# nanoporetech/medaka

Measured on NVIDIA H100. Metric: pileup positions/sec (consensus inference), higher is better.
Workload: dtype f32

## Files before the change

### medaka_b200/csrc/gru_wg.cu

```cuda
#include "common.cuh"
#include "ptx.cuh"
#include "rec_common.cuh"

namespace mdk {

constexpr int RW_THREADS = 256;
constexpr int RW_ABLK = (H / 8) * 64 * 16;
constexpr int RW_XBLK = 2 * 64 * 16;

template <int NT, bool FUSE_X, int OUT>
struct RwCfg {
    static constexpr int N = NT * RT_N;
    static constexpr bool HL = NT == 1;
    static constexpr int ROWS = HL ? 2 * N : N;
    static constexpr int PLANES = HL ? 1 : 2;
    static constexpr int KG = ROWS * 16 + 16;
    static_assert(KG % 16 == 0, "stmatrix rows are 16-byte aligned");
    static constexpr int HPLANE = (H / 8) * KG;
    static constexpr int XPLANE = 2 * KG;
    static constexpr int HLO = HL ? N * 16 : HPLANE;
    static constexpr int XLO = HL ? N * 16 : XPLANE;
    static constexpr int RED = (RW_THREADS / 32) * NCLS * N;
    static constexpr int wlo_off = 0;
    static constexpr int wxlo_off = wlo_off + 6 * RW_ABLK;
    static constexpr int h_off = wxlo_off + (FUSE_X ? 6 * RW_XBLK : 0);
    static constexpr int x_off = h_off + 2 * PLANES * HPLANE;
    static constexpr int red_off = x_off + (FUSE_X ? 2 * PLANES * XPLANE : 0);
    static constexpr int total = red_off + (OUT == OUT_LOGITS ? 2 * RED * 4 : 0);
    static_assert(total <= 227 * 1024, "smem budget");
};

__device__ __forceinline__ uint32_t ld_u32(const __half *p) { return *reinterpret_cast<const uint32_t *>(p); }

template <int NT, bool FUSE_X, int OUT>
__global__ void __launch_bounds__(RW_THREADS, 1)
rec_tc_kernel(const float *__restrict__ gi, RecX xin, const __half *__restrict__ w_hh, const float *__restrict__ b_hn,
              void *__restrict__ h_out, int64_t B, int64_t T, const float *__restrict__ lin_w,
              float *__restrict__ plog) {
    using L = RwCfg<NT, FUSE_X, OUT>;
    constexpr int N = L::N, NA = N / 2;
    constexpr int NACC = L::ROWS / 2;
    constexpr int NX = FUSE_X ? NACC : NA;
    using MMA = Wgmma<N>;
    using MMA_H = Wgmma<L::ROWS>;
    constexpr bool LOGITS = OUT == OUT_LOGITS;
    extern __shared__ __align__(128) uint8_t smem[];
    const int tid = threadIdx.x, wg = tid >> 7, warp = (tid >> 5) & 3, lane = tid & 31;
    const int gq = lane >> 2, cq = lane & 3;
    const int dir = blockIdx.y;
    const int64_t ntiles = (B + RT_N - 1) / RT_N;
    const int64_t wtile0 = (int64_t)blockIdx.x * NT;
    const int j0 = wg * 64 + warp * 16 + gq;
    const uint32_t sbase = smem_u32(smem);

    for (int i = tid; i < (L::total - L::h_off) / 16; i += RW_THREADS)
        reinterpret_cast<int4 *>(smem + L::h_off)[i] = make_int4(0, 0, 0, 0);
    for (int i = tid; i < 3 * H * (H / 8); i += RW_THREADS) {
        const int kg = i & 15, r = (i >> 4) & (H - 1), gate = i >> 11;
        const uint4 v = *reinterpret_cast<const uint4 *>(w_hh + ((((size_t)dir * 2 + 1) * 3 + gate) * H + r) * H + kg * 8);
        *reinterpret_cast<uint4 *>(smem + L::wlo_off + (gate * 2 + (r >> 6)) * RW_ABLK + kg * 1024 + (r & 63) * 16) = v;
    }
    if (FUSE_X) {
        for (int i = tid; i < 3 * H * 2; i += RW_THREADS) {
            const int kg = i & 1, r = (i >> 1) & (H - 1), gate = i >> 8;
            const uint4 v = *reinterpret_cast<const uint4 *>(xin.w_x + ((((size_t)dir * 2 + 1) * 3 + gate) * H + r) * 16 + kg * 8);
            *reinterpret_cast<uint4 *>(smem + L::wxlo_off + (gate * 2 + (r >> 6)) * RW_XBLK + kg * 1024 + (r & 63) * 16) = v;
        }
    }
    float wlin[2][NCLS];
    if (LOGITS) {
#pragma unroll
        for (int hb = 0; hb < 2; ++hb)
#pragma unroll
            for (int c = 0; c < NCLS; ++c) wlin[hb][c] = lin_w[c * H2 + dir * H + j0 + 8 * hb];
    }
    uint32_t whi[3][H / 16][4];
#pragma unroll
    for (int gate = 0; gate < 3; ++gate)
#pragma unroll
        for (int ks = 0; ks < H / 16; ++ks) {
            const __half *w = w_hh + ((((size_t)dir * 2) * 3 + gate) * H + j0) * H + ks * 16 + 2 * cq;
            whi[gate][ks][0] = ld_u32(w);
            whi[gate][ks][1] = ld_u32(w + 8 * H);
            whi[gate][ks][2] = ld_u32(w + 8);
            whi[gate][ks][3] = ld_u32(w + 8 * H + 8);
        }
    uint32_t wxhi[3][4];
    float bx[3][2] = {};
    if (FUSE_X) {
#pragma unroll
        for (int gate = 0; gate < 3; ++gate) {
            const __half *w = xin.w_x + ((((size_t)dir * 2) * 3 + gate) * H + j0) * 16 + 2 * cq;
            wxhi[gate][0] = ld_u32(w);
            wxhi[gate][1] = ld_u32(w + 8 * 16);
            wxhi[gate][2] = ld_u32(w + 8);
            wxhi[gate][3] = ld_u32(w + 8 * 16 + 8);
            bx[gate][0] = xin.bias[dir * G3 + gate * H + j0];
            bx[gate][1] = xin.bias[dir * G3 + gate * H + j0 + 8];
        }
    }
    const float bhn[2] = {b_hn[dir * H + j0], b_hn[dir * H + j0 + 8]};
    const uint32_t hst_addr = sbase + L::h_off + (lane >> 4) * L::HLO + (wg * 8 + warp * 2 + ((lane >> 3) & 1)) * L::KG +
                              (lane & 7) * 16;

    float ar[NACC], az[NACC], an[NACC], axn[NX], hp[NA];
#pragma unroll
    for (int k = 0; k < NA; ++k) hp[k] = 0.f;
    const float *gi_thr = FUSE_X ? nullptr
                                 : gi + wtile0 * T * GI_TS_FLOATS + ((dir * 3 * 4 + (cq >> 1)) * H + j0) * 4 + 2 * (cq & 1);
    auto load_pre = [&](int64_t t) {
#pragma unroll
        for (int i = 0; i < N / 8; ++i)
#pragma unroll
            for (int hb = 0; hb < 2; ++hb) {
                float2 v[3] = {make_float2(0.f, 0.f), make_float2(0.f, 0.f), make_float2(0.f, 0.f)};
                if (FUSE_X) {
#pragma unroll
                    for (int gate = 0; gate < 3; ++gate) v[gate] = make_float2(bx[gate][hb], bx[gate][hb]);
                } else if (i < 2 || wtile0 + (i >> 1) < ntiles) {
                    const float *p = gi_thr + ((i >> 1) * T + t) * GI_TS_FLOATS + (2 * (i & 1) * H + 8 * hb) * 4;
#pragma unroll
                    for (int gate = 0; gate < 3; ++gate) v[gate] = __ldcs(reinterpret_cast<const float2 *>(p + gate * 16 * H));
                }
                const int k = 4 * i + 2 * hb;
                ar[k] = v[0].x; ar[k + 1] = v[0].y;
                az[k] = v[1].x; az[k + 1] = v[1].y;
                axn[k] = v[2].x; axn[k + 1] = v[2].y;
                an[k] = bhn[hb]; an[k + 1] = bhn[hb];
            }
        if constexpr (L::HL) {
#pragma unroll
            for (int k = NA; k < NACC; ++k) {
                ar[k] = 0.f; az[k] = 0.f; an[k] = 0.f;
                if constexpr (FUSE_X) axn[k] = 0.f;
            }
        }
    };
    const int xF = FUSE_X ? xin.F : 1;
    const float *xsrc[NT];
    int xoff[NT];
    float xreg[NT];
#pragma unroll
    for (int m = 0; m < NT; ++m) {
        const int q = tid + RW_THREADS * m, xn = q / xF, xf = q - xn * xF;
        const bool own = FUSE_X && q < N * xF;
        xoff[m] = own ? (xf >> 3) * L::KG + xn * 16 + (xf & 7) * 2 : -1;
        xsrc[m] = (own && wtile0 * RT_N + xn < B) ? xin.feats + ((wtile0 * RT_N + xn) * T) * xF + xf : nullptr;
        xreg[m] = 0.f;
    }
    auto stage_x = [&](int buf, int m, float v) {
        __half hi, lo;
        split_f16(v, hi, lo);
        *reinterpret_cast<__half *>(smem + L::x_off + buf * L::PLANES * L::XPLANE + xoff[m]) = hi;
        *reinterpret_cast<__half *>(smem + L::x_off + buf * L::PLANES * L::XPLANE + L::XLO + xoff[m]) = lo;
    };
    const int64_t t_first = dir ? T - 1 : 0;
    if (FUSE_X) {
#pragma unroll
        for (int m = 0; m < NT; ++m) {
            if (xoff[m] < 0) continue;
            stage_x(0, m, xsrc[m] ? xsrc[m][t_first * xF] : 0.f);
        }
    }
    load_pre(t_first);
    fence_proxy_async_smem();
    __syncthreads();

    constexpr int NW = N / 4;
    auto head_partials = [&](int rb) {
        float v[NW][NCLS];
#pragma unroll
        for (int wl = 0; wl < NW; ++wl) {
            const int k = 4 * (wl >> 1) + (wl & 1);
#pragma unroll
            for (int c = 0; c < NCLS; ++c) v[wl][c] = fmaf(wlin[1][c], hp[k + 2], wlin[0][c] * hp[k]);
        }
        int wbase = 0;
#pragma unroll
        for (int lvl = 0; lvl < 3; ++lvl) {
            const int mask = 16 >> lvl;
            const int half = (NW >> lvl) / 2;
            if (half > 0) {
                const bool up = lane & mask;
#pragma unroll
                for (int w = 0; w < NW / 2; ++w) {
                    if (w >= half) continue;
#pragma unroll
                    for (int c = 0; c < NCLS; ++c) {
                        const float send = up ? v[w][c] : v[w + half][c];
                        const float keep = up ? v[w + half][c] : v[w][c];
                        v[w][c] = keep + __shfl_xor_sync(0xffffffffu, send, mask);
                    }
                }
                if (up) wbase += half;
            } else {
#pragma unroll
                for (int c = 0; c < NCLS; ++c) v[0][c] += __shfl_xor_sync(0xffffffffu, v[0][c], mask);
            }
        }
        if (NW >= 8 || !(lane & 4)) {
            float *red = reinterpret_cast<float *>(smem + L::red_off) + rb * L::RED + (tid >> 5) * NCLS * N;
            const int n = 8 * (wbase >> 1) + 2 * cq + (wbase & 1);
#pragma unroll
            for (int c = 0; c < NCLS; ++c) red[c * N + n] = v[0][c];
        }
    };
    auto head_store = [&](int rb, int64_t t) {
        if (tid >= NCLS * N) return;
        const int c = tid / N, n = tid % N;
        const float *red = reinterpret_cast<const float *>(smem + L::red_off) + rb * L::RED + c * N + n;
        float s = red[0];
#pragma unroll
        for (int w = 1; w < RW_THREADS / 32; ++w) s += red[w * NCLS * N];
        const int64_t wt = wtile0 + n / RT_N;
        if (wt < ntiles) plog[((dir * ntiles + wt) * T + t) * PLOG_TS_FLOATS + c * RT_N + (n & 15)] = s;
    };
    auto store_h0 = [&](int b, int64_t t) {
#pragma unroll
        for (int r = 0; r < NT * 512 / RW_THREADS; ++r) {
            const int q = tid + RW_THREADS * r, row = q & 15, kg = (q >> 4) & 15, p = (q >> 8) & 1, m = q >> 9;
            const int64_t wt = wtile0 + m;
            if (wt >= ntiles) continue;
            const int64_t orow = (wt * T + t) * RT_N + row;
            const int4 v = *reinterpret_cast<const int4 *>(smem + L::h_off + b * L::PLANES * L::HPLANE + p * L::HLO + kg * L::KG +
                                                           (m * RT_N + row) * 16);
            *reinterpret_cast<int4 *>(reinterpret_cast<uint8_t *>(h_out) + (orow >> 7) * (int64_t)XT_TILE_BYTES +
                                      p * XT_PLANE_BYTES + (dir * (H / 8) + kg) * (XT_ROWS * 16) + (orow & (XT_ROWS - 1)) * 16) = v;
        }
    };

#pragma unroll 1
    for (int64_t step = 0; step < T; ++step) {
        const int64_t t = dir ? T - 1 - step : step;
        const int buf = (int)(step & 1);
        const uint32_t hb_addr = sbase + L::h_off + buf * L::PLANES * L::HPLANE;
        wg_fence();
        if constexpr (L::HL) {
#pragma unroll
            for (int ks = 0; ks < H / 16; ++ks) {
                const uint64_t bh = make_smem_desc(hb_addr + ks * 2 * L::KG, L::KG, 128);
#pragma unroll
                for (int gate = 0; gate < 3; ++gate) MMA_H::rs(gate == 0 ? ar : (gate == 1 ? az : an), whi[gate][ks], bh, 1u);
#pragma unroll
                for (int gate = 0; gate < 3; ++gate)
                    MMA::ss(gate == 0 ? ar : (gate == 1 ? az : an),
                            make_smem_desc(sbase + L::wlo_off + (gate * 2 + wg) * RW_ABLK + ks * 2 * 1024, 1024, 128), bh, 1u);
            }
        } else {
#pragma unroll
            for (int ks = 0; ks < H / 16; ++ks) {
                const uint64_t bh = make_smem_desc(hb_addr + ks * 2 * L::KG, L::KG, 128);
                const uint64_t bl = make_smem_desc(hb_addr + L::HPLANE + ks * 2 * L::KG, L::KG, 128);
#pragma unroll
                for (int gate = 0; gate < 3; ++gate) MMA::rs(gate == 0 ? ar : (gate == 1 ? az : an), whi[gate][ks], bh, 1u);
#pragma unroll
                for (int gate = 0; gate < 3; ++gate) MMA::rs(gate == 0 ? ar : (gate == 1 ? az : an), whi[gate][ks], bl, 1u);
#pragma unroll
                for (int gate = 0; gate < 3; ++gate)
                    MMA::ss(gate == 0 ? ar : (gate == 1 ? az : an),
                            make_smem_desc(sbase + L::wlo_off + (gate * 2 + wg) * RW_ABLK + ks * 2 * 1024, 1024, 128), bh, 1u);
            }
        }
        if constexpr (FUSE_X) {
            const uint32_t xa = sbase + L::x_off + buf * L::PLANES * L::XPLANE;
            const uint64_t bh = make_smem_desc(xa, L::KG, 128);
            if constexpr (L::HL) {
#pragma unroll
                for (int gate = 0; gate < 3; ++gate) MMA_H::rs(gate == 0 ? ar : (gate == 1 ? az : axn), wxhi[gate], bh, 1u);
#pragma unroll
                for (int gate = 0; gate < 3; ++gate)
                    MMA::ss(gate == 0 ? ar : (gate == 1 ? az : axn),
                            make_smem_desc(sbase + L::wxlo_off + (gate * 2 + wg) * RW_XBLK, 1024, 128), bh, 1u);
            } else {
                const uint64_t bl = make_smem_desc(xa + L::XPLANE, L::KG, 128);
#pragma unroll
                for (int gate = 0; gate < 3; ++gate) MMA::rs(gate == 0 ? ar : (gate == 1 ? az : axn), wxhi[gate], bh, 1u);
#pragma unroll
                for (int gate = 0; gate < 3; ++gate) MMA::rs(gate == 0 ? ar : (gate == 1 ? az : axn), wxhi[gate], bl, 1u);
#pragma unroll
                for (int gate = 0; gate < 3; ++gate)
                    MMA::ss(gate == 0 ? ar : (gate == 1 ? az : axn),
                            make_smem_desc(sbase + L::wxlo_off + (gate * 2 + wg) * RW_XBLK, 1024, 128), bh, 1u);
            }
        }
        wg_commit();
        if (FUSE_X && step + 1 < T) {
#pragma unroll
            for (int m = 0; m < NT; ++m)
                if (xsrc[m]) xreg[m] = xsrc[m][(dir ? t - 1 : t + 1) * xF];
        }
        if (OUT == OUT_TILES && step > 0) store_h0(buf, dir ? t + 1 : t - 1);
        if (!FUSE_X && tid == 0 && step + GI_PREFETCH_STEPS < T) {
            const int64_t tp = dir ? t - GI_PREFETCH_STEPS : t + GI_PREFETCH_STEPS;
#pragma unroll
            for (int m = 0; m < NT; ++m) {
                if (wtile0 + m >= ntiles) break;
                const float *blk = gi + ((wtile0 + m) * T + tp) * GI_TS_FLOATS + (int64_t)dir * (GI_TS_FLOATS / 2);
#pragma unroll
                for (int i = 0; i < 12; ++i) bulk_prefetch_l2(blk + i * 512, 2048);
            }
        }
        if (LOGITS && step > 0) {
            if (step > 1) head_store((int)((step - 1) & 1), dir ? t + 2 : t - 2);
            head_partials((int)(step & 1));
        }
        wg_wait_all();
        wg_hold(ar); wg_hold(az); wg_hold(an); wg_hold(axn);

#pragma unroll
        for (int k = 0; k < NA; ++k) {
            float pr = ar[k], pz = az[k], pn = an[k], px = axn[k];
            if constexpr (L::HL) {
                pr += ar[k + NA]; pz += az[k + NA]; pn += an[k + NA];
                if constexpr (FUSE_X) px += axn[k + NA];
            }
            const float a = 1.f + ex2_approx(fminf(pr, EXP_CLAMP)), b = 1.f + ex2_approx(fminf(pz, EXP_CLAMP));
            const float q = rcp_approx(a * b);
            const float r = b * q, z = a * q;
            const float en = ex2_approx(fminf(fmaf(r, pn, px), EXP_CLAMP));
            const float n = (en - 1.f) * rcp_approx(en + 1.f);
            hp[k] = fmaf(z, hp[k] - n, n);
        }
#pragma unroll
        for (int i = 0; i < N / 8; ++i) {
            uint32_t hi[2], lo[2];
#pragma unroll
            for (int hb = 0; hb < 2; ++hb) split_f16x2(hp[4 * i + 2 * hb], hp[4 * i + 2 * hb + 1], hi[hb], lo[hb]);
            stmatrix_x4_trans(hst_addr + (buf ^ 1) * L::PLANES * L::HPLANE + i * 128, hi[0], hi[1], lo[0], lo[1]);
        }
        if (FUSE_X && step + 1 < T) {
#pragma unroll
            for (int m = 0; m < NT; ++m) {
                if (xoff[m] < 0) continue;
                stage_x(buf ^ 1, m, xreg[m]);
            }
        }
        if (OUT == OUT_ROWS) {
#pragma unroll
            for (int k = 0; k < NA; ++k) {
                const int i = k >> 2, n = 8 * i + 2 * cq + (k & 1);
                const int64_t wt = wtile0 + (i >> 1);
                if (wt >= ntiles) continue;
                const int64_t orow = (wt * T + t) * RT_N + (n & 15);
                reinterpret_cast<float *>(h_out)[orow * H2 + dir * H + j0 + 8 * ((k >> 1) & 1)] = hp[k];
            }
        }
        if (FUSE_X || step + 1 < T) load_pre(dir ? t - 1 : t + 1);
        fence_proxy_async_smem();
        __syncthreads();
    }
    if (OUT == OUT_TILES) store_h0((int)(T & 1), dir ? 0 : T - 1);
    if (LOGITS) {
        if (T > 1) head_store((int)((T - 1) & 1), dir ? 1 : T - 2);
        head_partials((int)(T & 1));
        __syncthreads();
        head_store((int)(T & 1), dir ? 0 : T - 1);
    }
}

template <int NT, bool FX, int OUT>
static cudaError_t launch_rec(const float *gi, const RecX &xin, const __half *w_hh_tm, const float *b_hn, void *out,
                              const float *lin_w, int64_t B, int64_t T, cudaStream_t s) {
    auto kern = rec_tc_kernel<NT, FX, OUT>;
    constexpr int smem_bytes = RwCfg<NT, FX, OUT>::total;
    cudaError_t e = cudaFuncSetAttribute(kern, cudaFuncAttributeMaxDynamicSharedMemorySize, smem_bytes);
    if (e != cudaSuccess) return e;
    const int64_t tiles = (B + RT_N - 1) / RT_N;
    dim3 grid((unsigned)((tiles + NT - 1) / NT), NDIR);
    constexpr bool LOGITS = OUT == OUT_LOGITS;
    kern<<<grid, RW_THREADS, smem_bytes, s>>>(gi, xin, w_hh_tm, b_hn, LOGITS ? nullptr : out, B, T, lin_w,
                                              LOGITS ? static_cast<float *>(out) : nullptr);
    return cudaGetLastError();
}

template <int NT>
static cudaError_t launch_rec_nt(const float *gi, const RecX *xin, const __half *w_hh_tm, const float *b_hn, int out_kind,
                                 void *out, const float *lin_w, int64_t B, int64_t T, cudaStream_t s) {
    if (xin)
        return out_kind == OUT_TILES ? launch_rec<NT, true, OUT_TILES>(gi, *xin, w_hh_tm, b_hn, out, nullptr, B, T, s)
                                     : cudaErrorInvalidValue;
    const RecX none{nullptr, nullptr, nullptr, 0};
    switch (out_kind) {
    case OUT_TILES: return launch_rec<NT, false, OUT_TILES>(gi, none, w_hh_tm, b_hn, out, nullptr, B, T, s);
    case OUT_ROWS: return launch_rec<NT, false, OUT_ROWS>(gi, none, w_hh_tm, b_hn, out, nullptr, B, T, s);
    case OUT_LOGITS:
        return lin_w ? launch_rec<NT, false, OUT_LOGITS>(gi, none, w_hh_tm, b_hn, out, lin_w, B, T, s) : cudaErrorInvalidValue;
    }
    return cudaErrorInvalidValue;
}

cudaError_t launch_rec_tc(const float *gi, const RecX *xin, const __half *w_hh_tm, const float *b_hn, int tiles_per_cta,
                          int out_kind, void *out, const float *lin_w, int64_t B, int64_t T, cudaStream_t s) {
    if (B == 0 || T == 0) return cudaSuccess;
    switch (tiles_per_cta) {
    case 1: return launch_rec_nt<1>(gi, xin, w_hh_tm, b_hn, out_kind, out, lin_w, B, T, s);
    case 2: return launch_rec_nt<2>(gi, xin, w_hh_tm, b_hn, out_kind, out, lin_w, B, T, s);
    }
    return cudaErrorInvalidValue;
}

constexpr int GW_THREADS = 256;
constexpr int GW_QK = 8;
constexpr int GW_STAGE_PLANE = GW_QK * XT_ROWS * 16;
constexpr int GW_STAGE = 2 * GW_STAGE_PLANE;
constexpr int GW_NQ = XT_K / 8 / GW_QK;
constexpr int GW_KS = XT_K / 16;
constexpr int GW_TS = XT_ROWS / WT;
constexpr int GW_QUAD = H * 4;
constexpr int GW_QUAD_PAD = GW_QUAD + 16;
constexpr int GW_OUT_OFF = GW_NQ * GW_STAGE;
constexpr int GW_BAR_OFF = GW_OUT_OFF + GW_TS * 4 * GW_QUAD_PAD * 4;
constexpr int GW_SMEM = GW_BAR_OFF + 2 * GW_NQ * 8;
static_assert(GW_SMEM <= 227 * 1024, "smem budget");
static_assert(GW_TS * 4 == 32, "one bulk store per lane of warp 0");

__global__ void __launch_bounds__(GW_THREADS, 1)
gemm_tc_kernel(const uint8_t *__restrict__ x_tiles, const __half *__restrict__ w_in_tm, const float *__restrict__ bias,
               float *__restrict__ gi, int64_t P, int64_t ntiles) {
    extern __shared__ __align__(128) uint8_t smem[];
    uint64_t *full = reinterpret_cast<uint64_t *>(smem + GW_BAR_OFF), *empty = full + GW_NQ;
    float *stg = reinterpret_cast<float *>(smem + GW_OUT_OFF);
    const int tid = threadIdx.x, wg = tid >> 7, warp = (tid >> 5) & 3, lane = tid & 31;
    const int gq = lane >> 2, cq = lane & 3;
    const int blk = blockIdx.x;
    const int j0 = wg * 64 + warp * 16 + gq;
    const uint32_t sbase = smem_u32(smem);
    const int64_t my_tiles = blockIdx.y < ntiles ? (ntiles - 1 - blockIdx.y) / gridDim.y + 1 : 0;
    auto issue = [&](int64_t n, int q) {
        const uint8_t *src = x_tiles + (blockIdx.y + n * gridDim.y) * (int64_t)XT_TILE_BYTES + q * GW_STAGE_PLANE;
        mbar_arrive_expect_tx(&full[q], GW_STAGE);
        bulk_g2s(smem + q * GW_STAGE, src, GW_STAGE_PLANE, &full[q]);
        bulk_g2s(smem + q * GW_STAGE + GW_STAGE_PLANE, src + XT_PLANE_BYTES, GW_STAGE_PLANE, &full[q]);
    };
    if (tid == 0) {
        for (int q = 0; q < GW_NQ; ++q) {
            mbar_init(&full[q], 1);
            mbar_init(&empty[q], GW_THREADS / 32);
        }
        fence_mbar_init();
        if (my_tiles > 0)
            for (int q = 0; q < GW_NQ; ++q) issue(0, q);
    }
    uint32_t wa[2][GW_KS][4];
#pragma unroll
    for (int p = 0; p < 2; ++p)
#pragma unroll
        for (int ks = 0; ks < GW_KS; ++ks) {
            const __half *w = w_in_tm + (((size_t)blk * 2 + p) * H + j0) * H2 + ks * 16 + 2 * cq;
            wa[p][ks][0] = ld_u32(w);
            wa[p][ks][1] = ld_u32(w + 8 * H2);
            wa[p][ks][2] = ld_u32(w + 8);
            wa[p][ks][3] = ld_u32(w + 8 * H2 + 8);
        }
    const float bj[2] = {bias[blk * H + j0], bias[blk * H + j0 + 8]};
    const uint64_t policy = l2_evict_first_policy();
    __syncthreads();
    auto release = [&](int64_t n, int q) {
        if (lane == 0) mbar_arrive(&empty[q]);
        if (tid == 0 && n + 1 < my_tiles) {
            mbar_wait(&empty[q], (uint32_t)(n & 1));
            issue(n + 1, q);
        }
        __syncwarp();
    };
    float acc[64];
#pragma unroll 1
    for (int64_t n = 0; n < my_tiles; ++n) {
#pragma unroll
        for (int q = 0; q < GW_NQ; ++q) {
            mbar_wait(&full[q], (uint32_t)(n & 1));
            wg_fence();
#pragma unroll
            for (int prod = 0; prod < 3; ++prod) {
                const int pa = prod == 2, pb = prod == 1;
#pragma unroll
                for (int kk = 0; kk < GW_QK / 2; ++kk) {
                    const uint64_t b = make_smem_desc(sbase + q * GW_STAGE + pb * GW_STAGE_PLANE + 2 * kk * (XT_ROWS * 16),
                                                      XT_ROWS * 16, 128);
                    Wgmma<128>::rs(acc, wa[pa][q * (GW_QK / 2) + kk], b, (q | prod | kk) ? 1u : 0u);
                }
            }
            wg_commit();
            if (q > 0) {
                wg_wait_1();
                release(n, q - 1);
            }
        }
        wg_wait_all();
        wg_hold(acc);
        release(n, GW_NQ - 1);

        const int64_t tile = blockIdx.y + n * gridDim.y;
        const int64_t prem = P - tile * XT_ROWS;
        if (tid < 32) bulk_wait_read_all();
        __syncthreads();
#pragma unroll
        for (int k = 0; k < 64; k += 2) {
            const int i = k >> 2, hb = (k >> 1) & 1;
            float *o = stg + ((i >> 1) * 4 + 2 * (i & 1) + (cq >> 1)) * GW_QUAD_PAD + (j0 + 8 * hb) * 4 + 2 * (cq & 1);
            *reinterpret_cast<float2 *>(o) = make_float2(acc[k] + bj[hb], acc[k + 1] + bj[hb]);
        }
        fence_proxy_async_smem();
        __syncthreads();
        if (tid < 32) {
            const int ts = lane >> 2, cg = lane & 3;
            if (ts * WT < prem)
                bulk_s2g(gi + (((tile * GW_TS + ts) * 6 + blk) * 4 + cg) * GW_QUAD, stg + lane * GW_QUAD_PAD,
                         GW_QUAD * 4, policy);
            bulk_commit();
        }
    }
    if (tid < 32) bulk_wait_all();
}

cudaError_t launch_gemm_tc(const void *x_tiles, const __half *w_in_tm, const float *bias, float *gi, int64_t P,
                           int sm_count, cudaStream_t s) {
    if (P == 0) return cudaSuccess;
    const int64_t ntiles = (P + XT_ROWS - 1) / XT_ROWS;
    cudaError_t ea = cudaFuncSetAttribute(gemm_tc_kernel, cudaFuncAttributeMaxDynamicSharedMemorySize, GW_SMEM);
    if (ea != cudaSuccess) return ea;
    int64_t ct = sm_count / 6;
    if (ct < 1) ct = 1;
    if (ct > ntiles) ct = ntiles;
    dim3 grid(6, (unsigned)ct);
    gemm_tc_kernel<<<grid, GW_THREADS, GW_SMEM, s>>>(reinterpret_cast<const uint8_t *>(x_tiles), w_in_tm, bias, gi, P, ntiles);
    return cudaGetLastError();
}

__global__ void __launch_bounds__(256, 1)
selftest_kernel(const float *__restrict__ A, const float *__restrict__ Bm, float *__restrict__ D, int N, int K) {
    extern __shared__ __align__(128) uint8_t smem[];
    const int a_plane = 128 * K * 2, b_plane = N * K * 2;
    uint8_t *sa = smem, *sb = smem + 2 * a_plane;
    const int tid = threadIdx.x, wg = tid >> 7, warp = (tid >> 5) & 3, lane = tid & 31;
    for (int i = tid; i < 128 * K; i += 256) {
        const int r = i / K, k = i % K;
        __half hi, lo;
        split_f16(A[i], hi, lo);
        const int off = (k / 8) * (128 * 16) + r * 16 + (k % 8) * 2;
        *reinterpret_cast<__half *>(sa + off) = hi;
        *reinterpret_cast<__half *>(sa + a_plane + off) = lo;
    }
    for (int i = tid; i < N * K; i += 256) {
        const int r = i / K, k = i % K;
        __half hi, lo;
        split_f16(Bm[i], hi, lo);
        const int off = (k / 8) * (N * 16) + r * 16 + (k % 8) * 2;
        *reinterpret_cast<__half *>(sb + off) = hi;
        *reinterpret_cast<__half *>(sb + b_plane + off) = lo;
    }
    fence_proxy_async_smem();
    __syncthreads();
    for (int n0 = 0; n0 < N; n0 += 16) {
        float d[8];
        wg_fence();
        uint32_t acc = 0;
        for (int prod = 0; prod < 3; ++prod) {
            const int pa = (prod == 2), pb = (prod == 1);
            for (int ks = 0; ks < K / 16; ++ks) {
                const uint64_t ad = make_smem_desc(smem_u32(sa + pa * a_plane) + ks * 2 * 128 * 16 + wg * 64 * 16, 128 * 16, 128);
                const uint64_t bd = make_smem_desc(smem_u32(sb + pb * b_plane) + ks * 2 * N * 16 + n0 * 16, N * 16, 128);
                Wgmma<16>::ss(d, ad, bd, acc);
                acc = 1;
            }
        }
        wg_commit();
        wg_wait_all();
        wg_hold(d);
        const int row = wg * 64 + warp * 16 + (lane >> 2);
        for (int k = 0; k < 8; ++k)
            D[(row + 8 * ((k >> 1) & 1)) * N + n0 + 8 * (k >> 2) + 2 * (lane & 3) + (k & 1)] = d[k];
    }
}

int selftest_umma(int device, const float *A, const float *B, float *D, int N, int K, int variant) {
    MDK_REQUIRE(N >= 16 && N <= 128 && N % 16 == 0, MDK_ERR_ARG, "selftest_umma: N must be a multiple of 16 in [16,128]");
    MDK_REQUIRE(K >= 16 && K <= 256 && K % 16 == 0, MDK_ERR_ARG, "selftest_umma: K must be a multiple of 16 in [16,256]");
    MDK_REQUIRE(variant == 0, MDK_ERR_ARG, "selftest_umma: variant must be 0");
    MDK_CUDA(cudaSetDevice(device));
    float *dA = nullptr, *dB = nullptr, *dD = nullptr;
    MDK_CUDA(cudaMalloc(&dA, sizeof(float) * 128 * K));
    MDK_CUDA(cudaMalloc(&dB, sizeof(float) * N * K));
    MDK_CUDA(cudaMalloc(&dD, sizeof(float) * 128 * N));
    MDK_CUDA(cudaMemcpy(dA, A, sizeof(float) * 128 * K, cudaMemcpyHostToDevice));
    MDK_CUDA(cudaMemcpy(dB, B, sizeof(float) * N * K, cudaMemcpyHostToDevice));
    const int smem = 2 * 128 * K * 2 + 2 * N * K * 2;
    MDK_REQUIRE(smem <= 227 * 1024, MDK_ERR_ARG, "selftest_umma: N*K too large for shared memory");
    MDK_CUDA(cudaFuncSetAttribute(selftest_kernel, cudaFuncAttributeMaxDynamicSharedMemorySize, smem));
    selftest_kernel<<<1, 256, smem>>>(dA, dB, dD, N, K);
    MDK_CUDA(cudaGetLastError());
    MDK_CUDA(cudaDeviceSynchronize());
    MDK_CUDA(cudaMemcpy(D, dD, sizeof(float) * 128 * N, cudaMemcpyDeviceToHost));
    cudaFree(dA); cudaFree(dB); cudaFree(dD);
    return MDK_OK;
}

}
```

Measured before the change: 187.0 million.

## Replace per-step block barrier with per-warpgroup mbarriers split over K halves

Replaces the end-of-step __syncthreads with mbarriers that each warpgroup arrives on once its half of the new hidden state is written. The next step waits on the first half's barrier, issues the first half of the K-loop MMAs, then waits on the second half's barrier, so the two warpgroups can run out of lockstep. store_h0 and head_store are reassigned so each warpgroup handles its own data, the GI L2 prefetch becomes a single bulk request, and the prefetch moves to a thread in the second warpgroup. This risks correctness hazards around buffer reuse, since the reads of the shared red and h buffers by the other warpgroup are no longer covered by a full barrier.

New measurement: 190.8 million, median of 6. +2.0%, better.

```diff
diff --git a/medaka_b200/csrc/gru_wg.cu b/medaka_b200/csrc/gru_wg.cu
--- a/medaka_b200/csrc/gru_wg.cu
+++ b/medaka_b200/csrc/gru_wg.cu
@@ -26,7 +26,8 @@
     static constexpr int h_off = wxlo_off + (FUSE_X ? 6 * RW_XBLK : 0);
     static constexpr int x_off = h_off + 2 * PLANES * HPLANE;
     static constexpr int red_off = x_off + (FUSE_X ? 2 * PLANES * XPLANE : 0);
-    static constexpr int total = red_off + (OUT == OUT_LOGITS ? 2 * RED * 4 : 0);
+    static constexpr int bar_off = red_off + (OUT == OUT_LOGITS ? 2 * RED * 4 : 0);
+    static constexpr int total = bar_off + 4 * 8;
     static_assert(total <= 227 * 1024, "smem budget");
 };
 
@@ -53,8 +54,11 @@
     const int j0 = wg * 64 + warp * 16 + gq;
     const uint32_t sbase = smem_u32(smem);
 
-    for (int i = tid; i < (L::total - L::h_off) / 16; i += RW_THREADS)
+    for (int i = tid; i < (L::bar_off - L::h_off) / 16; i += RW_THREADS)
         reinterpret_cast<int4 *>(smem + L::h_off)[i] = make_int4(0, 0, 0, 0);
+    uint64_t *hready = reinterpret_cast<uint64_t *>(smem + L::bar_off);
+    if (tid == 0)
+        for (int i = 0; i < 4; ++i) mbar_init(&hready[i], RW_THREADS / 2);
     for (int i = tid; i < 3 * H * (H / 8); i += RW_THREADS) {
         const int kg = i & 15, r = (i >> 4) & (H - 1), gate = i >> 11;
         const uint4 v = *reinterpret_cast<const uint4 *>(w_hh + ((((size_t)dir * 2 + 1) * 3 + gate) * H + r) * H + kg * 8);
@@ -206,8 +210,9 @@
         }
     };
     auto head_store = [&](int rb, int64_t t) {
-        if (tid >= NCLS * N) return;
-        const int c = tid / N, n = tid % N;
+        const int q = tid - (RW_THREADS - NCLS * N);
+        if (q < 0) return;
+        const int c = q / N, n = q % N;
         const float *red = reinterpret_cast<const float *>(smem + L::red_off) + rb * L::RED + c * N + n;
         float s = red[0];
 #pragma unroll
@@ -217,8 +222,8 @@
     };
     auto store_h0 = [&](int b, int64_t t) {
 #pragma unroll
-        for (int r = 0; r < NT * 512 / RW_THREADS; ++r) {
-            const int q = tid + RW_THREADS * r, row = q & 15, kg = (q >> 4) & 15, p = (q >> 8) & 1, m = q >> 9;
+        for (int r = 0; r < NT * 2; ++r) {
+            const int q = (tid & 127) + 128 * r, row = q & 15, kg = wg * 8 + ((q >> 4) & 7), p = (q >> 7) & 1, m = q >> 8;
             const int64_t wt = wtile0 + m;
             if (wt >= ntiles) continue;
             const int64_t orow = (wt * T + t) * RT_N + row;
@@ -229,38 +234,39 @@
         }
     };
 
+    auto mma_h = [&](uint32_t hb_addr, int ks0) {
+#pragma unroll
+        for (int kk = 0; kk < H / 32; ++kk) {
+            const int ks = ks0 + kk;
+            const uint64_t bh = make_smem_desc(hb_addr + ks * 2 * L::KG, L::KG, 128);
+            if constexpr (L::HL) {
+#pragma unroll
+                for (int gate = 0; gate < 3; ++gate) MMA_H::rs(gate == 0 ? ar : (gate == 1 ? az : an), whi[gate][ks], bh, 1u);
+            } else {
+                const uint64_t bl = make_smem_desc(hb_addr + L::HPLANE + ks * 2 * L::KG, L::KG, 128);
+#pragma unroll
+                for (int gate = 0; gate < 3; ++gate) MMA::rs(gate == 0 ? ar : (gate == 1 ? az : an), whi[gate][ks], bh, 1u);
+#pragma unroll
+                for (int gate = 0; gate < 3; ++gate) MMA::rs(gate == 0 ? ar : (gate == 1 ? az : an), whi[gate][ks], bl, 1u);
+            }
+#pragma unroll
+            for (int gate = 0; gate < 3; ++gate)
+                MMA::ss(gate == 0 ? ar : (gate == 1 ? az : an),
+                        make_smem_desc(sbase + L::wlo_off + (gate * 2 + wg) * RW_ABLK + ks * 2 * 1024, 1024, 128), bh, 1u);
+        }
+    };
+
 #pragma unroll 1
     for (int64_t step = 0; step < T; ++step) {
         const int64_t t = dir ? T - 1 - step : step;
         const int buf = (int)(step & 1);
         const uint32_t hb_addr = sbase + L::h_off + buf * L::PLANES * L::HPLANE;
+        const uint32_t par = (uint32_t)((step - 1) >> 1) & 1u;
+        if (step > 0) mbar_wait(&hready[buf * 2], par);
         wg_fence();
-        if constexpr (L::HL) {
-#pragma unroll
-            for (int ks = 0; ks < H / 16; ++ks) {
-                const uint64_t bh = make_smem_desc(hb_addr + ks * 2 * L::KG, L::KG, 128);
-#pragma unroll
-                for (int gate = 0; gate < 3; ++gate) MMA_H::rs(gate == 0 ? ar : (gate == 1 ? az : an), whi[gate][ks], bh, 1u);
-#pragma unroll
-                for (int gate = 0; gate < 3; ++gate)
-                    MMA::ss(gate == 0 ? ar : (gate == 1 ? az : an),
-                            make_smem_desc(sbase + L::wlo_off + (gate * 2 + wg) * RW_ABLK + ks * 2 * 1024, 1024, 128), bh, 1u);
-            }
-        } else {
-#pragma unroll
-            for (int ks = 0; ks < H / 16; ++ks) {
-                const uint64_t bh = make_smem_desc(hb_addr + ks * 2 * L::KG, L::KG, 128);
-                const uint64_t bl = make_smem_desc(hb_addr + L::HPLANE + ks * 2 * L::KG, L::KG, 128);
-#pragma unroll
-                for (int gate = 0; gate < 3; ++gate) MMA::rs(gate == 0 ? ar : (gate == 1 ? az : an), whi[gate][ks], bh, 1u);
-#pragma unroll
-                for (int gate = 0; gate < 3; ++gate) MMA::rs(gate == 0 ? ar : (gate == 1 ? az : an), whi[gate][ks], bl, 1u);
-#pragma unroll
-                for (int gate = 0; gate < 3; ++gate)
-                    MMA::ss(gate == 0 ? ar : (gate == 1 ? az : an),
-                            make_smem_desc(sbase + L::wlo_off + (gate * 2 + wg) * RW_ABLK + ks * 2 * 1024, 1024, 128), bh, 1u);
-            }
-        }
+        mma_h(hb_addr, 0);
+        if (step > 0) mbar_wait(&hready[buf * 2 + 1], par);
+        mma_h(hb_addr, H / 32);
         if constexpr (FUSE_X) {
             const uint32_t xa = sbase + L::x_off + buf * L::PLANES * L::XPLANE;
             const uint64_t bh = make_smem_desc(xa, L::KG, 128);
@@ -290,14 +296,13 @@
                 if (xsrc[m]) xreg[m] = xsrc[m][(dir ? t - 1 : t + 1) * xF];
         }
         if (OUT == OUT_TILES && step > 0) store_h0(buf, dir ? t + 1 : t - 1);
-        if (!FUSE_X && tid == 0 && step + GI_PREFETCH_STEPS < T) {
+        if (!FUSE_X && tid == RW_THREADS / 2 && step + GI_PREFETCH_STEPS < T) {
             const int64_t tp = dir ? t - GI_PREFETCH_STEPS : t + GI_PREFETCH_STEPS;
 #pragma unroll
             for (int m = 0; m < NT; ++m) {
                 if (wtile0 + m >= ntiles) break;
-                const float *blk = gi + ((wtile0 + m) * T + tp) * GI_TS_FLOATS + (int64_t)dir * (GI_TS_FLOATS / 2);
-#pragma unroll
-                for (int i = 0; i < 12; ++i) bulk_prefetch_l2(blk + i * 512, 2048);
+                bulk_prefetch_l2(gi + ((wtile0 + m) * T + tp) * GI_TS_FLOATS + (int64_t)dir * (GI_TS_FLOATS / 2),
+                                 GI_TS_FLOATS / 2 * 4);
             }
         }
         if (LOGITS && step > 0) {
@@ -347,8 +352,9 @@
         }
         if (FUSE_X || step + 1 < T) load_pre(dir ? t - 1 : t + 1);
         fence_proxy_async_smem();
-        __syncthreads();
-    }
+        mbar_arrive(&hready[(buf ^ 1) * 2 + wg]);
+    }
+    if (OUT != OUT_ROWS) __syncthreads();
     if (OUT == OUT_TILES) store_h0((int)(T & 1), dir ? 0 : T - 1);
     if (LOGITS) {
         if (T > 1) head_store((int)((T - 1) & 1), dir ? 1 : T - 2);
```
